# epruesse/metacov

Hardware: AMD Instinct MI355X
Metric: aligned bases/sec into per-position depth vector, 1/2/4/8 MI355X (higher is better)
Workload: dtype int32

## Files before the change

### metacov_amd/csrc/engine.hip

```cpp
#include <hip/hip_ext.h>
#include <hip/hip_runtime.h>

#include <algorithm>
#include <atomic>
#include <cmath>
#include <cstdlib>
#include <cstring>
#include <vector>

#include "../../include/metacov_amd.h"
#include "common.h"
#include "kernels.h"
#include "npstd.h"
#include "capmask.h"

#include <hipcub/hipcub.hpp>

using namespace mc;

#ifndef MC_PLAIN_TILES_PER_CHUNK
#define MC_PLAIN_TILES_PER_CHUNK 4
#endif
constexpr int kPlainTilesPerChunk = MC_PLAIN_TILES_PER_CHUNK;

// ... 105 lines not shown
        hipError_t e = hipHostMalloc(&h, n, hipHostMallocDefault);
        if (e == hipSuccess) cap = n;
        else h = nullptr;
        return e;
    }
    void release() {
        if (h) (void)hipHostFree(h);
        h = nullptr;
        cap = 0;
    }
};

}

struct mc_ctx {
    int device = 0;
    hipStream_t stream = nullptr;
    bool own_stream = false;

    std::vector<int64_t> len, extent, coff;
    DevBuf<int64_t> d_len, d_coff;
    std::vector<int64_t> coff_dev;
    uint64_t coff_dev_gen = ~0ull;

    int64_t n_reads = 0;
    DevBuf<int32_t> d_tid, d_pos, d_span;
    DevBuf<uint32_t> d_gpos;
    bool spans_pending = false;
    DevBuf<int64_t> d_cig_off;
    DevBuf<uint32_t> d_cigar;
    const int64_t* cig_off_ext = nullptr;
    const uint32_t* cigar_ext = nullptr;

    bool prepared = false;
    bool direct = false;
    bool direct_checked = false;
    bool direct_ok = true;
    bool direct_enabled = true;
    int min_span = 0;
    bool direct_retry_full = false;
    unsigned long long direct_gen = 0;
    int direct_halo = 0;
    int direct_halo_used = 0;
    DevBuf<int32_t> d_jidx;
    DevBuf<int32_t> d_fsamp;
    DevBuf<unsigned long long> d_dres;
// ... 53 lines not shown
        int64_t chunk_w = 0, n_chunks = 0;
        std::vector<int64_t> extent, coff;
    } fcache;
    DevBuf<unsigned> d_flow;
    DevBuf<unsigned> d_fhist;
    HostMapped<int> h_fflag;
    DevBuf<unsigned> d_fb_hist;
    DevBuf<RegionAcc> d_fb_acc;
    DevBuf<int32_t> d_fb_list;
    DevBuf<unsigned> d_fb_cnt;
    DevBuf<unsigned> d_kdone;
    int64_t fb_calls = 0;
    bool fb_recent = false;
    int64_t device_recomputes = 0;
    bool fused_clean = false;
    int64_t fused_clean_R = 0;
    bool check_clean = false;
    DevBuf<unsigned long long> d_check;
    int64_t fused_fallbacks = 0;

    hipEvent_t ev[8] = {};
    struct TimingSet {
        hipEvent_t e[4] = {};
        bool prep = false;
        bool pending = false;
    };
    static constexpr int kTimingSets = 4;
    TimingSet ts[kTimingSets];
    int ts_cur = 0;
    HostMapped<unsigned long long> h_done;
    unsigned long long done_seq = 0;
    bool stamp_ok = true;
    int ingest_grid[2] = {0, 0};
    int k2_resident[6] = {};
    size_t k2_resident_lds[6] = {};
    mc_timings t{};
    bool t_cigar = false, t_prep = false, t_depth = false, t_stats = false;
};

static int ctx_use(mc_ctx* ctx) {
    MC_REQUIRE(ctx, MC_E_INVALID, "null ctx");
    HIP_TRY(hipSetDevice(ctx->device));
    return MC_OK;
}

static void invalidate(mc_ctx* ctx) {
    ctx->prepared = false;
    ctx->direct = false;
    ctx->direct_checked = false;
// ... 102 lines not shown
    if (s) {
        ctx->stream = (hipStream_t)s;
        ctx->own_stream = false;
    } else {
        HIP_TRY(hipStreamCreateWithFlags(&ctx->stream, hipStreamNonBlocking));
        ctx->own_stream = true;
    }
    return MC_OK;
}

extern "C" int mc_ctx_device(const mc_ctx* ctx, int* device) {
    MC_REQUIRE(ctx && device, MC_E_INVALID, "null argument");
    *device = ctx->device;
    return MC_OK;
}

extern "C" int mc_set_contigs(mc_ctx* ctx, int32_t n, const int64_t* lengths) {
    if (int rc = ctx_use(ctx)) return rc;
    MC_REQUIRE(n >= 0 && (n == 0 || lengths), MC_E_INVALID, "bad contig table");
    for (int32_t i = 0; i < n; ++i)
        MC_REQUIRE(lengths[i] >= 0 && lengths[i] < (int64_t(1) << 40), MC_E_INVALID,
                   "contig %d: bad length %lld", i, (long long)lengths[i]);
    ctx->len.assign(lengths, lengths + n);
    ctx->direct_ok = true;
    ctx->long_hint = false;
    ctx->n_reads = 0;
    ctx->spans_pending = false;
    ctx->cig_off_ext = nullptr;
    ctx->cigar_ext = nullptr;
    invalidate(ctx);
    HIP_TRY(ctx->d_len.reserve(std::max<int64_t>(n, 1)));
    if (n) HIP_TRY(hipMemcpy(ctx->d_len.p, lengths, n * sizeof(int64_t), hipMemcpyHostToDevice));
    return MC_OK;
}

static int reserve_reads(mc_ctx* ctx, int64_t n_total, bool cigar_mode) {
    const size_t cap = (size_t)round_up(n_total + kPadBatch, kPadBatch);
    if (cap > ctx->d_tid.cap) {
        size_t ncap = std::max(cap, ctx->d_tid.cap * 3 / 2);
        ncap = (size_t)round_up((int64_t)ncap, kPadBatch);
        DevBuf<int32_t> t2, p2, s2;
        HIP_TRY(t2.reserve(ncap));
        HIP_TRY(p2.reserve(ncap));
        HIP_TRY(s2.reserve(ncap));
        if (ctx->n_reads) {
            HIP_TRY(hipMemcpyAsync(t2.p, ctx->d_tid.p, ctx->n_reads * 4, hipMemcpyDeviceToDevice, ctx->stream));
// ... 138 lines not shown
#define MC_STEP_EVENTS 1
#endif
#ifndef MC_EXT_EVENTS
#define MC_EXT_EVENTS 0
#endif
static float elapsed(hipEvent_t a, hipEvent_t b) {
    float ms = 0.f;
    if (hipEventElapsedTime(&ms, a, b) != hipSuccess) {
        (void)hipGetLastError();
        return 0.f;
    }
    return ms;
}

static float elapsed(mc_ctx* ctx, int a, int b) { return elapsed(ctx->ev[a], ctx->ev[b]); }

static void resolve_prepare_timing(mc_ctx* ctx) {
    if (!ctx->prep_pending || hipEventQuery(ctx->ev[3]) != hipSuccess) return;
    ctx->t.prepare_ms = elapsed(ctx, 2, 3);
    ctx->t.prepare_ms_total += ctx->t.prepare_ms;
    ctx->prep_pending = false;
}

static void resolve_timings(mc_ctx* ctx, bool all) {
    for (int i = 1; i <= mc_ctx::kTimingSets; ++i) {
        const int k = (ctx->ts_cur + i) % mc_ctx::kTimingSets;
        auto& T = ctx->ts[k];
        if (!T.pending || (k == ctx->ts_cur && !all)) continue;
        const float a = elapsed(T.e[1], T.e[2]), b = elapsed(T.e[2], T.e[3]);
        ctx->t.fused_depth_ms_total += a;
        ctx->t.fused_stats_ms_total += b;
        ctx->t.depth_ms = a;
        ctx->t.stats_ms = b;
        if (T.prep) {
            ctx->t.prepare_ms = elapsed(T.e[0], T.e[1]);
            ctx->t.prepare_ms_total += ctx->t.prepare_ms;
        }
        T.prep = T.pending = false;
    }
}

#ifndef MC_MIN_CHUNKS
#define MC_MIN_CHUNKS 2048
#endif
static void set_layout(mc_ctx* ctx, const std::vector<int64_t>& ext) {
    const int32_t nc = (int32_t)ctx->len.size();
    ctx->extent = ext;
    ctx->coff.resize(nc + 1);
    int64_t off = 0;
    for (int32_t i = 0; i < nc; ++i) {
        ctx->coff[i] = off;
        off += round_up(ext[i], 64);
    }
    ctx->coff[nc] = off;
    ctx->total_len = off;
    const int64_t tiles = std::max<int64_t>(1, (off + kTileW - 1) / kTileW);
    const int top = ctx->long_hint ? kTilesPerChunkLong : kTilesPerChunk;
    const int min_tpc = (kRing % kTileW == 0) ? kRing / kTileW : top;
    int tpc = top;
    while (tpc / 2 >= min_tpc && tpc % 2 == 0 && tiles / tpc < MC_MIN_CHUNKS &&
           ((int64_t)(tpc / 2) * kTileW) % kRing == 0)
        tpc /= 2;
    ctx->tiles_per_chunk = tpc;
    ctx->chunk_w = (int64_t)tpc * kTileW;
    ctx->n_chunks = std::max<int64_t>(1, (off + ctx->chunk_w - 1) / ctx->chunk_w);
    int tpc_base = tpc;
    if (tpc > kPlainTilesPerChunk && tpc % kPlainTilesPerChunk == 0 &&
        ((int64_t)kPlainTilesPerChunk * kTileW) % kRing == 0)
        tpc_base = kPlainTilesPerChunk;
// ... 209 lines not shown
        HIP_TRY(hipStreamSynchronize(s));
        ctx->t.cigar_ms = elapsed(ctx, 0, 1);
    } else if (ctx->t_cigar) {
        ctx->t.cigar_ms = elapsed(ctx, 0, 1);
    }
    ctx->prep_pending = true;
    ctx->prepared = true;
    ctx->depth_valid = false;
    ++ctx->prep_gen;
    ctx->t.full_prepares += 1;
    return MC_OK;
}

static bool direct_eligible(const mc_ctx* ctx) {
    return ctx->direct_enabled && ctx->direct_ok && ctx->n_reads > 0 && !ctx->len.empty();
}

static int prepare_direct(mc_ctx* ctx) {
    const int32_t nc = (int32_t)ctx->len.size();
    const int64_t n = ctx->n_reads;
    hipStream_t s = ctx->stream;
    if (int rc = run_k1(ctx)) return rc;
    auto& T = ctx->ts[ctx->ts_cur];
    if (MC_STEP_EVENTS && !MC_EXT_EVENTS) HIP_TRY(hipEventRecord(T.e[0], s));
    T.prep = true;
    ctx->ring = kRing;
    ctx->short_max = ctx->ring - kTileW;
    const size_t n_res = 8 + 2 * (size_t)nc;
    HIP_TRY(ctx->pin_io.reserve((n_res + nc + 1) * 8));
    int64_t* coff_up = reinterpret_cast<int64_t*>(static_cast<unsigned long long*>(ctx->pin_io.h) + n_res);
    set_layout(ctx, ctx->len);
    if (int rc = upload_coff(ctx, coff_up)) return rc;
    const int64_t n_base = ctx->n_chunks * ctx->cstride;
    HIP_TRY(ctx->d_jidx.reserve(3 * (n_base + 1)));
    HIP_TRY(ctx->d_fsamp.reserve(nc + 1));
    if (!ctx->d_dres.p) {
        HIP_TRY(ctx->d_dres.reserve(kDresWords));
        HIP_TRY(hipMemsetAsync(ctx->d_dres.p, 0, kDresWords * 8, s));
    }
    ctx->direct_halo_used = ctx->direct_halo > 0 ? std::min(ctx->direct_halo, ctx->short_max) : ctx->short_max;
    ProbeArgs P{ctx->d_tid.p, ctx->d_pos.p, ctx->d_span.p, n, nc, ctx->d_coff.p, base_lw(ctx),
                ctx->short_max, ctx->direct_halo_used, n_base, ctx->d_jidx.p, ctx->d_jidx.p + (n_base + 1),
                ctx->d_jidx.p + 2 * (n_base + 1), ctx->d_fsamp.p,
                ctx->d_dres.p, ++ctx->direct_gen};
    const int64_t M = (n + kProbeStride - 1) >> kProbeShift;
    hipExtLaunchKernelGGL(probe_kernel, dim3((unsigned)std::max<int64_t>(1, (M + kBlock - 1) / kBlock)),
                          dim3(kBlock), 0, s, MC_STEP_EVENTS && MC_EXT_EVENTS ? T.e[0] : nullptr, nullptr, 0, P);
    HIP_TRY(hipGetLastError());
    HIP_TRY(ctx->d_depth.reserve((size_t)(ctx->n_chunks * ctx->chunk_w)));
    ctx->has_long = false;
    ctx->max_span = 0;
    ctx->aligned_bases = -1;
    ctx->prepared = true;
    ctx->direct = true;
    ctx->direct_checked = false;
    ctx->depth_valid = false;
    ++ctx->prep_gen;
    return MC_OK;
}

static int next_halo(unsigned long long max_span, int short_max) {
    const long long h = round_up((long long)max_span + (long long)max_span / 8, 64);
    return (int)std::max<long long>(64, std::min<long long>(h, short_max));
}

static bool check_direct(mc_ctx* ctx, const unsigned long long* res, bool deferred = false) {
    const unsigned long long g = ctx->direct_gen;
    if (res[kDresBadSample] == g || res[kDresLongSample] == g || res[kDresFlags] ||
        res[kDresMaxSpan] > (unsigned long long)ctx->direct_halo_used)
        return false;
    ctx->max_span = (int32_t)res[kDresMaxSpan];
    ctx->direct_halo = next_halo(res[kDresMaxSpan], ctx->short_max);
    ctx->aligned_bases = -1;
    ctx->direct_checked = true;
    ctx->t.direct_batches += 1;
    auto& T = ctx->ts[ctx->ts_cur];
    if (!deferred && T.prep) {
        ctx->t.prepare_ms = elapsed(T.e[0], ctx->ev[4]);
        ctx->t.prepare_ms_total += ctx->t.prepare_ms;
        T.prep = false;
    }
    ctx->t.cigar_ms = ctx->t_cigar ? elapsed(ctx, 0, 1) : 0.f;
    return true;
}

static void direct_fallback(mc_ctx* ctx, const unsigned long long* res) {
    const unsigned long long g = ctx->direct_gen;
    const bool long_reads = res[kDresLongSample] == g || res[kDresMaxSpan] > (unsigned long long)ctx->short_max;
    if (long_reads || (res[kDresFlags] & kDirectUnfit)) ctx->direct_ok = false;
    if (long_reads || res[kDresBadSample] == g || res[kDresFlags]) {
        ctx->direct_retry_full = true;
    } else {
        ctx->direct_halo = next_halo(res[kDresMaxSpan], ctx->short_max);
        ctx->t.halo_redos += 1;
    }
    ctx->fused_clean = false;
    invalidate(ctx);
}

static int prepare_for_compute(mc_ctx* ctx) {
    if (ctx->prepared) return MC_OK;
// ... 62 lines not shown
              "K2Consts: padding beyond DirectArgs' 4 bytes after nc");
static int k2_consts(mc_ctx* ctx, const K2Consts& kc, const K2Consts** out) {
    for (int i = 0; i < mc_ctx::kK2Slots; ++i)
        if (ctx->k2c_valid[i] && std::memcmp(&ctx->k2c[i], &kc, sizeof kc) == 0) {
            *out = ctx->d_k2c.p + i;
            return MC_OK;
        }
    HIP_TRY(ctx->d_k2c.reserve(mc_ctx::kK2Slots));
    HIP_TRY(ctx->h_k2c.reserve(sizeof(K2Consts) * mc_ctx::kK2Slots));
    const int i = ctx->k2c_next;
    ctx->k2c_next = (i + 1) % mc_ctx::kK2Slots;
    if (ctx->k2c_ev[i]) HIP_TRY(hipEventSynchronize(ctx->k2c_ev[i]));
    else HIP_TRY(hipEventCreateWithFlags(&ctx->k2c_ev[i], hipEventDisableTiming));
    K2Consts* stage = reinterpret_cast<K2Consts*>(ctx->h_k2c.h) + i;
    std::memcpy(stage, &kc, sizeof kc);
    HIP_TRY(hipMemcpyAsync(ctx->d_k2c.p + i, stage, sizeof kc, hipMemcpyHostToDevice, ctx->stream));
    HIP_TRY(hipEventRecord(ctx->k2c_ev[i], ctx->stream));
    ctx->k2c[i] = kc;
    ctx->k2c_valid[i] = true;
    *out = ctx->d_k2c.p + i;
    return MC_OK;
}

static int launch_depth(mc_ctx* ctx, const FusedRegions& fr, hipEvent_t ea = nullptr, hipEvent_t eb = nullptr) {
    hipStream_t s = ctx->stream;
    const bool stats = fr.n > 0;
    const size_t lds = (size_t)(kLdsHeader + ctx->ring +
                                (stats ? (ctx->has_long ? HistCfg<true>::kLds : HistCfg<false>::kLds) + kOvInts
                                       : 0)) * 4;
    const bool lng = ctx->has_long;
    const bool dir = ctx->direct;
    const void* kfn = stats ? (lng ? (const void*)depth_kernel<true, true, false>
                                   : dir ? (const void*)depth_kernel<true, false, true>
                                         : (const void*)depth_kernel<true, false, false>)
                            : (lng ? (const void*)depth_kernel<false, true, false>
                                   : dir ? (const void*)depth_kernel<false, false, true>
                                         : (const void*)depth_kernel<false, false, false>);
    const K2Geom geo = k2_geom(ctx, stats);
    const int tpc = geo.tpc;
    const int64_t nch = geo.n_chunks;
    const int cstride = geo.cstride;
    const int64_t* cfirst = ctx->d_chunk_first.p;
    int grid = 0;
    if (int rc = occupancy_grid(ctx, (stats ? 1 : 0) + (lng ? 2 : dir ? 4 : 0), kfn, lds, nch, &grid))
        return rc;
    if (!stats) {
        ctx->fused_clean = false;
        HIP_TRY(hipMemsetAsync(ctx->d_queue.p, 0, 32, s));
        HIP_TRY(hipMemsetAsync(ctx->d_maxdepth.p, 0, 16, s));
    }
    hipEvent_t k2_start = MC_STEP_EVENTS || !ea ? (ea ? ea : ctx->ev[4]) : nullptr;
    hipEvent_t k2_stop = MC_STEP_EVENTS || !eb ? (eb ? eb : ctx->ev[5]) : nullptr;
    if (!MC_EXT_EVENTS && k2_start) HIP_TRY(hipEventRecord(k2_start, s));
    const int64_t* toff = ctx->has_long ? ctx->d_tile_off.p : nullptr;
    const int32_t* tev = ctx->has_long ? ctx->d_tile_ev.p : nullptr;
    const int* ccar = ctx->has_long ? ctx->d_chunk_carry.p : nullptr;
    const int64_t n_base = ctx->n_chunks * ctx->cstride;
    K2Consts kc;
    std::memset(&kc, 0, sizeof kc);
    kc.A = ReadArrays{ctx->d_gpos.p, ctx->d_tid.p, ctx->d_pos.p, ctx->d_span.p};
    kc.R = fr;
    DirectWindow w = direct_window(ctx);
    w.parity = 0;
    kc.D.j0 = ctx->d_jidx.p;
    kc.D.jh = ctx->d_jidx.p + (n_base + 1);
    kc.D.jn = ctx->d_jidx.p + 2 * (n_base + 1);
    kc.D.len = ctx->d_len.p;
    kc.D.nc = (int32_t)ctx->len.size();
    kc.D.dres = ctx->d_dres.p;
    kc.D.win = w;
    const K2Consts* dk = nullptr;
    if (int rc = k2_consts(ctx, kc, &dk)) return rc;
    const int win_parity = (int)(ctx->direct_gen & 1);
#define MC_LAUNCH_K2(S, L, D)                                                                  \
    hipExtLaunchKernelGGL((depth_kernel<S, L, D>), dim3(grid), dim3(kK2Block), (uint32_t)lds, s,        \
// ... 199 lines not shown

struct FusedLayout {
    size_t gs, ge, id, base, ntot, nzx, brow, rtid, rfused, up, total;
};
static FusedLayout fused_layout(int64_t nf, int64_t R) {
    auto al = stage_align;
    FusedLayout L;
    L.gs = 0;
    L.ge = L.gs + al(nf * 8);
    L.id = L.ge + al(nf * 8);
    L.base = L.id + al(nf * 4);
    L.ntot = L.base + al(nf * 4);
    L.nzx = L.ntot + al(R * 8);
    L.brow = L.nzx + al(R * 8);
    L.rtid = L.brow + al(R * 4);
    L.rfused = L.rtid + al(R * 4);
    L.up = L.rfused + al(R * 4);
    L.total = L.up;
    return L;
}

constexpr int kRedo = 1;

static size_t fflag_ints(int64_t R) { return (size_t)round_up(R + 1, 2) + 2 * kDresWords; }
static unsigned long long* fflag_dres(int* base, int64_t R) {
    return reinterpret_cast<unsigned long long*>(base + round_up(R + 1, 2));
}

static int direct_verdict_sync(mc_ctx* ctx) {
    if (!ctx->direct || ctx->direct_checked) return MC_OK;
    unsigned long long* res = static_cast<unsigned long long*>(ctx->pin_io.h);
    HIP_TRY(hipMemcpyAsync(res, ctx->d_dres.p, kDresWords * 8, hipMemcpyDeviceToHost, ctx->stream));
    HIP_TRY(hipStreamSynchronize(ctx->stream));
    if (check_direct(ctx, res)) return MC_OK;
    direct_fallback(ctx, res);
    return kRedo;
}

#ifndef MC_DONE_MODE
#define MC_DONE_MODE 1
#endif
static int wait_event_spin(hipEvent_t ev) {
    for (;;) {
        const hipError_t e = hipEventQuery(ev);
        if (e == hipSuccess) return MC_OK;
        if (e != hipErrorNotReady) HIP_TRY(e);
        __builtin_ia32_pause();
// ... 47 lines not shown
    } else if (ctx->check_clean) {
        HIP_TRY(ctx->d_check.reserve(1));
        HIP_TRY(hipMemsetAsync(ctx->d_check.p, 0, sizeof(unsigned long long), s));
        hipLaunchKernelGGL(fused_clean_check_kernel, dim3(1024), dim3(kBlock), 0, s, ctx->d_fhist.p, R * vals,
                           ctx->d_flow.p, ctx->d_acc.p, R, ctx->d_queue.p, ctx->d_maxdepth.p, ctx->d_check.p);
        HIP_TRY(hipGetLastError());
        unsigned long long bad = 0;
        HIP_TRY(hipMemcpyAsync(&bad, ctx->d_check.p, sizeof bad, hipMemcpyDeviceToHost, s));
        HIP_TRY(hipStreamSynchronize(s));
        MC_REQUIRE(bad == 0, MC_E_STATE, "fused buffers not initialised on a clean call (%llu words differ)", bad);
    }
    FusedRegions fr{nf,
                    ctx->d_fchunk.p,
                    reinterpret_cast<const int64_t*>(d + o_gs),
                    d_fge,
                    reinterpret_cast<const int32_t*>(d + o_id),
                    reinterpret_cast<const int32_t*>(d + o_base),
                    reinterpret_cast<const int32_t*>(d + L.rtid),
                    ctx->d_acc.p,
                    ctx->d_fhist.p,
                    ctx->d_flow.p};
    if (nf == 0) fr.n = 0;
    auto& T = ctx->ts[ctx->ts_cur];
    if (int rc = launch_depth(ctx, fr, T.e[1], T.e[2])) return rc;
    const unsigned long long seq = ++ctx->done_seq;
    unsigned long long* stamp = nullptr;
    if (ctx->stamp_ok) {
        if (!ctx->h_done.h) {
            if (ctx->h_done.reserve(1) != hipSuccess || ctx->d_kdone.reserve(1) != hipSuccess ||
                hipMemsetAsync(ctx->d_kdone.p, 0, sizeof(unsigned), s) != hipSuccess) {
                (void)hipGetLastError();
                ctx->stamp_ok = false;
            } else {
                __atomic_store_n(ctx->h_done.h, 0ull, __ATOMIC_RELEASE);
            }
        }
        if (ctx->stamp_ok && MC_DONE_MODE == 1) stamp = ctx->h_done.d;
    }
    const bool devfb = ctx->has_long || ctx->fb_recent;
    FbArgs F{};
    if (devfb) {
        if (!ctx->d_fb_cnt.p) {
            HIP_TRY(ctx->d_fb_hist.reserve((size_t)kFbSlots * kLdsBins));
            HIP_TRY(ctx->d_fb_acc.reserve(kFbSlots));
            HIP_TRY(ctx->d_fb_list.reserve(kFbSlots));
            HIP_TRY(ctx->d_fb_cnt.reserve(2));
            HIP_TRY(hipMemsetAsync(ctx->d_fb_cnt.p, 0, 8, s));
            hipLaunchKernelGGL(fused_init_kernel, dim3(1024), dim3(kBlock), 0, s, ctx->d_fb_hist.p,
                               (int64_t)kFbSlots * kLdsBins, (unsigned*)nullptr, ctx->d_fb_acc.p,
                               (int64_t)kFbSlots, (const int64_t*)nullptr, (int64_t)0, (int64_t)1, (int64_t)0,
                               (int64_t*)nullptr, (unsigned*)nullptr, (int*)nullptr);
            HIP_TRY(hipGetLastError());
        }
        F = FbArgs{ctx->d_depth.p,
                   reinterpret_cast<const int32_t*>(d + L.rfused),
                   reinterpret_cast<const int64_t*>(d + o_gs),
                   reinterpret_cast<const int64_t*>(d + o_ge),
                   reinterpret_cast<const int64_t*>(d + o_ntot),
                   reinterpret_cast<const int64_t*>(d + o_nzx),
                   ctx->h_fflag.d + R,
                   ctx->d_fb_list.p,
                   ctx->d_fb_cnt.p,
                   (int)(ctx->fb_calls & 1),
                   ctx->d_fb_hist.p,
                   ctx->d_fb_acc.p,
                   d_out};
        ctx->fb_calls += 1;
    }
    hipEvent_t k3_stop = MC_STEP_EVENTS && MC_EXT_EVENTS ? T.e[3] : nullptr;
#define MC_LAUNCH_K3B(V)                                                                           \
    hipExtLaunchKernelGGL(region_final_wave_kernel<V>, dim3((unsigned)((R + kWaves - 1) / kWaves)),     \
                          dim3(kBlock), 0u, s, nullptr, devfb ? nullptr : k3_stop, 0u,                   \
                          ctx->d_fhist.p, R, ctx->d_acc.p,                                              \
                       reinterpret_cast<const int64_t*>(d + o_ntot),                                \
                       reinterpret_cast<const int64_t*>(d + o_nzx), d_out, ctx->h_fflag.d,           \
                       reinterpret_cast<const int32_t*>(d + o_brow), ctx->d_flow.p,                 \
                       ctx->d_maxdepth.p, ctx->h_fflag.d + R, ctx->d_queue.p,                       \
                       verdict ? ctx->d_dres.p : nullptr, verdict ? fflag_dres(ctx->h_fflag.d, R) : nullptr, \
                       devfb ? F.cnt + F.parity : nullptr, devfb ? F.list : nullptr,                \
                       ctx->direct ? direct_window(ctx) : DirectWindow{},                          \
                       ctx->direct ? reinterpret_cast<const int32_t*>(d + L.rtid) : nullptr,           \
                       ctx->d_kdone.p, devfb ? nullptr : stamp, seq)
    if (vals == HistCfg<false>::kBins) MC_LAUNCH_K3B(HistCfg<false>::kBins);
    else MC_LAUNCH_K3B(HistCfg<true>::kBins);
#undef MC_LAUNCH_K3B
    HIP_TRY(hipGetLastError());
    if (devfb) {
        hipLaunchKernelGGL(fb_seg_kernel, dim3(1024), dim3(kBlock), (size_t)kLdsBins * 4, s, F);
        HIP_TRY(hipGetLastError());
        hipExtLaunchKernelGGL(fb_final_kernel, dim3(kFbSlots), dim3(kBlock), 0u, s, nullptr, k3_stop, 0u, F);
        HIP_TRY(hipGetLastError());
    }
    if (MC_STEP_EVENTS && !MC_EXT_EVENTS) HIP_TRY(hipEventRecord(T.e[3], s));
    if ((MC_DONE_MODE == 0 || (MC_DONE_MODE == 1 && devfb)) && ctx->stamp_ok && hipStreamWriteValue64(s, ctx->h_done.d, seq, 0) != hipSuccess) {
        (void)hipGetLastError();
        ctx->stamp_ok = false;
    }
    ctx->t_stats = false;
    ctx->t.stats_launches += 1;
    resolve_timings(ctx, false);
    if (int rc = MC_DONE_MODE == 2 ? wait_event_spin(T.e[3]) : wait_stamp(ctx, seq)) return rc;
    const int* flags = ctx->h_fflag.h;
    if (verdict && !check_direct(ctx, fflag_dres(ctx->h_fflag.h, R), true)) {
        direct_fallback(ctx, fflag_dres(ctx->h_fflag.h, R));
        T.prep = T.pending = false;
        return kRedo;
    }
    T.pending = true;
    ctx->ts_cur = (ctx->ts_cur + 1) % mc_ctx::kTimingSets;
    ctx->max_depth = flags[R];
    int64_t n_flag = 0;
    for (int64_t r = 0; r < R; ++r) n_flag += flags[r] ? 1 : 0;
    const bool on_device = devfb && n_flag <= kFbSlots && ctx->max_depth < kLdsBins;
    std::vector<int32_t> ft;
    std::vector<int64_t> fs, fe, fr_idx;
    if (!on_device)
        for (int64_t r = 0; r < R; ++r)
            if (flags[r]) {
                ft.push_back(tid[r]);
                fs.push_back(start[r]);
                fe.push_back(end[r]);
                fr_idx.push_back(r);
            }
    ctx->fused_fallbacks = (int64_t)ft.size();
    ctx->device_recomputes = on_device ? n_flag : 0;
    ctx->fb_recent = n_flag > 0;
    if (ft.empty()) {
        ctx->fused_clean = true;
        ctx->fused_clean_R = R;
    }
    if (!ft.empty()) {
        if (int rc = region_stats_impl(ctx, (int64_t)ft.size(), ft.data(), fs.data(), fe.data(),
                                       d_out, fr_idx.data()))
            return rc;
        HIP_TRY(hipEventSynchronize(ctx->ev[7]));
        ctx->t.fused_stats_ms_total += elapsed(ctx, 6, 7);
    }
    ctx->t.fused_calls += 1;
    return MC_OK;
}

static int depth_stats_once(mc_ctx* ctx, int64_t R, const int32_t* tid, const int64_t* start,
                            const int64_t* end, RegionOut* d_out) {
    if (int rc = prepare_for_compute(ctx)) return rc;
    MC_REQUIRE(R >= 0 && (R == 0 || (tid && start && end)), MC_E_INVALID, "bad region arrays");
    auto& fc = ctx->fcache;
    const bool direct = ctx->direct;
    const int vals = fused_hist_vals(ctx->has_long);
    const int64_t win_below = (int64_t)kWinBelow * vals / kHistBins;
    const double span_mean = ctx->n_reads ? (double)ctx->aligned_bases / (double)ctx->n_reads : 0.0;
    auto window_base = [&](int32_t t) {
        const int64_t ext = ctx->extent[t];
        const double body = ext > 2 * span_mean ? (double)ext - span_mean : (double)ext;
        const double depth_est = ext > 0 ? (double)ctx->cbases[t] / body : 0.0;
        return (int32_t)std::max<int64_t>(0, std::llrint(depth_est) - win_below);
    };
    const bool same = R > 0 && fc.valid && (int64_t)fc.tid.size() == R &&
                      std::memcmp(fc.tid.data(), tid, R * 4) == 0 &&
                      std::memcmp(fc.start.data(), start, R * 8) == 0 &&
                      std::memcmp(fc.end.data(), end, R * 8) == 0;
    if (same && fc.gen == ctx->prep_gen) return depth_stats_launch(ctx, R, tid, start, end, d_out, fc.nf);
    const K2Geom geo = k2_geom(ctx, true);
    if (same && fc.vals == vals && fc.chunk_w == geo.chunk_w && fc.n_chunks == geo.n_chunks &&
        fc.extent == ctx->extent && fc.coff == ctx->coff) {
        const FusedLayout L = fused_layout(fc.nf, R);
        if (!direct && R > 0) {
            const int32_t nc = (int32_t)ctx->len.size();
// ... 403 lines not shown
```

### metacov_amd/csrc/kernels.h

```cpp
#pragma once

#include <hip/hip_runtime.h>
#include <stdint.h>

namespace mc {

#ifndef MC_TILE_W
#define MC_TILE_W 4096
#endif
#ifndef MC_RING
#define MC_RING (2 * MC_TILE_W)
#endif
#ifndef MC_TILES_PER_CHUNK
#define MC_TILES_PER_CHUNK 8
#endif
#ifndef MC_PREFETCH
#define MC_PREFETCH 1
#endif
#ifndef MC_PREFETCH_STATS
#define MC_PREFETCH_STATS 1
#endif
#ifndef MC_APPLY_SHORT
#define MC_APPLY_SHORT 1
#endif
// ... 504 lines not shown
    if (threadIdx.x < 4) {
        long long v = red[threadIdx.x][0];
#pragma unroll
        for (int w = 1; w < kWaves; ++w)
            v = threadIdx.x == 3 ? max(v, red[3][w]) : v + red[threadIdx.x][w];
        if (threadIdx.x == 3) atomicMax(&out[3], (unsigned long long)v);
        else if (v) atomicAdd(&out[threadIdx.x], (unsigned long long)v);
    }
}

constexpr int kProbeShift = 8;
constexpr int kNearHalo = 256;
constexpr int kFarHaloMin = MC_FAR_HALO_MIN;
constexpr int kProbeStride = 1 << kProbeShift;

enum : int {
    kDresBadSample = 0,
    kDresLongSample = 1,
    kDresFlags = 2,
    kDresBases = 3,
    kDresMaxSpan = 4,
    kDresSpanSum = 5,
    kDresSpanCnt = 6,
    kDresWords = 9
};
constexpr unsigned kDirectInvalid = 1;
constexpr unsigned kDirectUnfit = 2;

struct ProbeArgs {
    const int32_t* tid;
    const int32_t* pos;
    const int32_t* span;
    int64_t n;
    int32_t nc;
    const int64_t* coff;
    int lw;
    int short_max;
    int halo;
    int64_t n_base;
    int32_t* j0;
    int32_t* jh;
    int32_t* jn;
    int32_t* fsamp;
    unsigned long long* dres;
    unsigned long long gen;
};

struct DirectWindow {
// ... 21 lines not shown

__device__ __forceinline__ int64_t probe_key(const ProbeArgs& A, int t, int p) {
    const int ct = t < 0 ? 0 : t >= A.nc ? A.nc - 1 : t;
    const int64_t k = A.coff[ct] + (int64_t)(p < 0 ? 0 : p);
    return k;
}

__device__ __forceinline__ void probe_fill(int32_t* J, int64_t n_base, int lw, int64_t off, int64_t key,
                                           int64_t key_next, bool first, bool last, int32_t val) {
    int64_t k0 = first ? 0 : ((key + off) >> lw) + 1;
    int64_t k1 = last ? n_base : ((key_next + off) >> lw);
    if (k1 > n_base) k1 = n_base;
    if (first) {
        int64_t kz = (key + off) >> lw;
        if (kz > n_base) kz = n_base;
        for (int64_t k = 0; k <= kz; ++k) J[k] = 0;
        k0 = kz + 1;
    }
    for (int64_t k = k0; k <= k1; ++k) J[k] = val;
}

constexpr int kProbeSpanEvery = 4;
constexpr unsigned kProbeMeanBlocks = 64;

__global__ void __launch_bounds__(kBlock)
probe_kernel(ProbeArgs A) {
    const int64_t M = (A.n + kProbeStride - 1) >> kProbeShift;
    const int64_t j = (int64_t)blockIdx.x * kBlock + threadIdx.x;
    const int par = (int)(A.gen & 1);
    if (blockIdx.x == 0 && threadIdx.x >= kDresFlags && threadIdx.x <= kDresMaxSpan) A.dres[threadIdx.x] = 0;
    if (blockIdx.x == 0 && threadIdx.x < 2) A.dres[kDresSpanSum + 2 * (par ^ 1) + threadIdx.x] = 0;
    const bool sampled = j < M && (j % kProbeSpanEvery) == 0;
    const int s0 = sampled ? A.span[j << kProbeShift] : 0;
    const unsigned every = max(1u, gridDim.x / kProbeMeanBlocks);
    if (blockIdx.x % every == 0) {
        __shared__ long long red[2 * kWaves];
        const bool s_ok = sampled && s0 >= 0;
        const long long wsum = wave_sum64(s_ok ? (long long)s0 : 0);
        const long long wcnt = wave_sum64(s_ok ? 1 : 0);
        if ((threadIdx.x & 63) == 0) {
            red[threadIdx.x >> 6] = wsum;
            red[kWaves + (threadIdx.x >> 6)] = wcnt;
        }
        __syncthreads();
        if (threadIdx.x == 0) {
            long long ts = 0, tc = 0;
#pragma unroll
            for (int w = 0; w < kWaves; ++w) {
                ts += red[w];
                tc += red[kWaves + w];
            }
            if (tc) {
                atomicAdd(&A.dres[kDresSpanSum + 2 * par], (unsigned long long)ts);
                atomicAdd(&A.dres[kDresSpanCnt + 2 * par], (unsigned long long)tc);
            }
        }
    }
    if (j >= M) return;
    const bool last = j == M - 1;
    const int64_t i = j << kProbeShift, i1 = last ? i : i + kProbeStride;
    const int t = A.tid[i], p = A.pos[i];
    const int t_next = A.tid[i1], p_next = A.pos[i1];
    const int s = s0;
    const int64_t key = probe_key(A, t, p);
    const int64_t key_next = probe_key(A, t_next, p_next);
    const bool bad = ((unsigned)t >= (unsigned)A.nc) | (p < 0) | (s < 0);
    const bool uns = !last && ((t > t_next) | ((t == t_next) & (p > p_next)) | (key > key_next));
    if (bad | uns) atomicMax(&A.dres[kDresBadSample], A.gen);
    if (s > A.short_max) atomicMax(&A.dres[kDresLongSample], A.gen);
    const bool first = j == 0;
    probe_fill(A.j0, A.n_base, A.lw, 0, key, key_next, first, last, (int32_t)(j + 1));
    probe_fill(A.jh, A.n_base, A.lw, A.halo, key, key_next, first, last, (int32_t)(j + 1));
    if (MC_FAR_HALO) probe_fill(A.jn, A.n_base, A.lw, kNearHalo, key, key_next, first, last, (int32_t)(j + 1));
    const int ct = t < 0 ? 0 : t >= A.nc ? A.nc - 1 : t;
    const int cn = last ? A.nc : (t_next < 0 ? 0 : t_next >= A.nc ? A.nc - 1 : t_next);
    if (first)
        for (int k = 0; k <= ct; ++k) A.fsamp[k] = 0;
    for (int k = ct + 1; k <= cn; ++k) A.fsamp[k] = (int32_t)(j + 1);
}

__global__ void __launch_bounds__(kBlock)
window_bases_kernel(const unsigned long long* __restrict__ ingest_out, const unsigned long long* __restrict__ cbases,
                    int64_t n, const int64_t* __restrict__ len, const int32_t* __restrict__ rtid,
                    const int32_t* __restrict__ rfused, int64_t R, int win_below, int32_t* __restrict__ brow,
                    int32_t* __restrict__ fbase) {
// ... 753 lines not shown
    unsigned f = a.flags;
    int m = a.max_span;
#pragma unroll
    for (int d = 32; d > 0; d >>= 1) {
        f |= __shfl_xor(f, d, 64);
        m = max(m, __shfl_xor(m, d, 64));
    }
    __syncthreads();
    if (lane == 0) {
        red[wave] = (int)f;
        red[kK2Waves + wave] = m;
    }
    __syncthreads();
    if (threadIdx.x == 0) {
        unsigned ff = 0;
        int mm = 0;
#pragma unroll
        for (int w = 0; w < kK2Waves; ++w) {
            ff |= (unsigned)red[w];
            mm = max(mm, red[kK2Waves + w]);
        }
        if (ff) atomicOr(&D.dres[kDresFlags], (unsigned long long)ff);
        if (mm > 0) atomicMax(&D.dres[kDresMaxSpan], (unsigned long long)mm);
    }
}

__global__ void __launch_bounds__(kBlock)
span_sum_kernel(const int32_t* __restrict__ span, int64_t n, unsigned long long* __restrict__ part) {
    long long s = 0;
    const int64_t n4 = n >> 2;
    const int64_t stride = (int64_t)gridDim.x * kBlock;
    int64_t i = (int64_t)blockIdx.x * kBlock + threadIdx.x;
    for (; i + 3 * stride < n4; i += 4 * stride) {
        i32x4 v[4];
#pragma unroll
        for (int u = 0; u < 4; ++u) v[u] = __builtin_nontemporal_load(reinterpret_cast<const i32x4*>(span) + i + u * stride);
#pragma unroll
        for (int u = 0; u < 4; ++u) s += (long long)v[u].x + v[u].y + v[u].z + v[u].w;
    }
    for (; i < n4; i += stride) {
        const i32x4 v = reinterpret_cast<const i32x4*>(span)[i];
        s += (long long)v.x + v.y + v.z + v.w;
    }
    if (blockIdx.x == 0 && threadIdx.x < (n & 3)) s += span[(n4 << 2) + threadIdx.x];
    s = wave_sum64(s);
    __shared__ long long ws[kWaves];
// ... 235 lines not shown
             int32_t* __restrict__ depth, unsigned* __restrict__ queue,
             int* __restrict__ max_depth, unsigned long long gen, int win_parity) {
    static_assert(!(kDirect && kLong), "the direct path has no long reads");
    const auto& KC = *(const __attribute__((address_space(4))) K2Consts*)K;
    const auto& R = KC.R;
    const auto& D = KC.D;
    extern __shared__ __attribute__((aligned(16))) int lds[];
    int* hdr = lds;
    int and_flip = 0;
    int* ring = lds + kLdsHeader;
    unsigned* hist = reinterpret_cast<unsigned*>(ring + kRing);
    using HC = HistCfg<kLong>;
    OvLds* ovf = reinterpret_cast<OvLds*>(hist + HC::kLds);
    const int lane = threadIdx.x & 63;
    unsigned* hist_lane = hist + (lane & (HC::kCopies - 1)) * HC::kStride;
    const int hist_dummy = HC::kBins + (lane / HC::kCopies) % HC::kPad;
    const int wave = __builtin_amdgcn_readfirstlane(threadIdx.x >> 6);
    const int64_t chunk_w = (int64_t)tiles_per_chunk * kTileW;
    constexpr int kWaveSpan = kTileW / kK2Waves;
    constexpr int kChunks = kWaveSpan / (64 * 4);
    constexpr bool kDefer = !kStats || (kLong && MC_DEFER_LONG) || (kDirect && MC_DEFER_DIRECT);
    constexpr bool kPf = kStats ? MC_PREFETCH_STATS : MC_PREFETCH;
    if (kDirect) {
        const unsigned long long f0 = uload(D.dres, kDresBadSample), f1 = uload(D.dres, kDresLongSample);
        if (f0 == gen || f1 == gen) return;
    }
    int my_max = 0;
    DirectAcc dacc;
    OvReg ovr;
    ov_reg_reset(ovr);
    if (kStats) {
        for (int k = threadIdx.x; k < HC::kLds; k += kK2Block) hist[k] = 0;
        if (threadIdx.x < kOvRecs) ov_reset(ovf + threadIdx.x);
    }

    constexpr bool kAhead = kStats && kLong;
    int ticket = 0;
    if (threadIdx.x == 0) hdr[0] = take_chunk(queue, n_chunks);
    const int ring_tail = (int)(((int64_t)tiles_per_chunk * kTileW) % kRing);
    for (int k = threadIdx.x * 4; k < kRing; k += kK2Block * 4)
        *reinterpret_cast<i32x4*>(ring + k) = i32x4{0, 0, 0, 0};
    for (;;) {
        __syncthreads();
        const int64_t c = (unsigned)__builtin_amdgcn_readfirstlane(hdr[0]);
        if (c >= n_chunks) break;
        if (kAhead && threadIdx.x == 0) ticket = take_chunk(queue, n_chunks);
// ... 555 lines not shown
            vmax = max(vmax, max(max(y0, y1), max(y2, y3)));
            vmin = min(vmin, min(min((unsigned)y0, (unsigned)y1), min((unsigned)y2, (unsigned)y3)));
        }
    }
}

struct FbArgs {
    const int32_t* depth;
    const int32_t* rfused;
    const int64_t* fgs;
    const int64_t* fge;
    const int64_t* ntot;
    const int64_t* nzx;
    const int* max_depth;
    int32_t* list;
    unsigned* cnt;
    int parity;
    unsigned* hist;
    RegionAcc* acc;
    RegionOut* out;
};

__device__ __forceinline__ void grid_done_stamp(unsigned* done_cnt, unsigned long long* stamp,
                                                unsigned long long seq) {
    if (stamp == nullptr) return;
    asm volatile("s_waitcnt vmcnt(0)" ::: "memory");
    __syncthreads();
    if (threadIdx.x == 0) {
        const unsigned prev = __hip_atomic_fetch_add(done_cnt, 1u, __ATOMIC_RELAXED, __HIP_MEMORY_SCOPE_AGENT);
        if (prev == gridDim.x - 1) {
            __hip_atomic_store(done_cnt, 0u, __ATOMIC_RELAXED, __HIP_MEMORY_SCOPE_AGENT);
            __builtin_amdgcn_fence(__ATOMIC_RELEASE, "");
            __hip_atomic_store(stamp, seq, __ATOMIC_RELAXED, __HIP_MEMORY_SCOPE_SYSTEM);
        }
    }
}

template <class T>
__device__ __forceinline__ void store_sys(T* p, T v) {
    __hip_atomic_store(p, v, __ATOMIC_RELAXED, __HIP_MEMORY_SCOPE_SYSTEM);
}

__global__ void __launch_bounds__(kBlock)
fb_seg_kernel(FbArgs F) {
    extern __shared__ __attribute__((aligned(16))) unsigned hb[];
    const int n = (int)min(F.cnt[F.parity], (unsigned)kFbSlots);
    const int maxd = *F.max_depth;
    if (n == 0 || maxd >= kLdsBins) return;
    const int nb = maxd + 1;
    const int per = max(1, (int)gridDim.x / n);
    __shared__ int ext[2 * kWaves];
    for (int w = blockIdx.x; w < n * per; w += gridDim.x) {
        const int i = w / per, part = w % per;
        const int k = F.rfused[F.list[i]];
// ... 46 lines not shown
        F.acc[b].min = 0x7fffffff;
        F.acc[b].max = 0;
    }
}

__global__ void __launch_bounds__(kBlock)
fb_final_kernel(FbArgs F) {
    fb_final_row(F);
}

template <int kVals>
__device__ __forceinline__ void
final_wave_row(unsigned* __restrict__ hist, int64_t R,
               RegionAcc* __restrict__ acc, const int64_t* __restrict__ n_total,
               const int64_t* __restrict__ n_zero_extra, RegionOut* __restrict__ out,
               int* __restrict__ fallback, const int32_t* __restrict__ base_of,
               unsigned* __restrict__ low_of, int* __restrict__ max_depth,
               int* __restrict__ max_out, unsigned* __restrict__ queue,
               const unsigned long long* __restrict__ dres_in, unsigned long long* __restrict__ dres_out,
               unsigned* __restrict__ fb_cnt, int32_t* __restrict__ fb_list,
               DirectWindow dwin, const int32_t* __restrict__ rtid, bool wt) {
    constexpr int kFinPer = (kVals + 63) / 64;
    const int lane = threadIdx.x & 63;
    if (blockIdx.x == 0 && dres_out && threadIdx.x < kDresWords) {
        if (wt) store_sys(dres_out + threadIdx.x, dres_in[threadIdx.x]);
        else dres_out[threadIdx.x] = dres_in[threadIdx.x];
    }
    if (blockIdx.x == 0 && threadIdx.x == 0) {
        if (max_out) {
            if (wt) store_sys(max_out, *max_depth);
            else *max_out = *max_depth;
        }
        if (queue) {
            for (int k = 0; k < 4; ++k) max_depth[k] = 0;
            for (int k = 0; k < 8; ++k) queue[k] = 0;
        }
    }
    const int64_t r = (int64_t)blockIdx.x * kWaves + (threadIdx.x >> 6);
    if (r >= R) return;
    unsigned* hr = hist + r * kVals;
    const long long n = n_total[r];
    const long long zx = n_zero_extra[r];
    const long long base = rtid ? direct_window_base(dwin, dwin.parity, __builtin_amdgcn_readfirstlane(rtid[r]))
                                : base_of[r];
    const long long zx_bin = base == 0 ? zx : 0;
    const long long low = (long long)low_of[r] + (base == 0 ? 0 : zx);
    const long long r_lo = (n - 1) / 2, r_hi = n / 2;
// ... 98 lines not shown
        const unsigned long long* v = reinterpret_cast<const unsigned long long*>(&o);
#pragma unroll
        for (int k = 0; k < (int)(sizeof(RegionOut) / 8); ++k) store_sys(w + k, v[k]);
    } else {
        out[r] = o;
    }
}

template <int kVals>
__global__ void __launch_bounds__(kBlock)
region_final_wave_kernel(unsigned* __restrict__ hist, int64_t R,
                         RegionAcc* __restrict__ acc, const int64_t* __restrict__ n_total,
                         const int64_t* __restrict__ n_zero_extra, RegionOut* __restrict__ out,
                         int* __restrict__ fallback, const int32_t* __restrict__ base_of,
                         unsigned* __restrict__ low_of, int* __restrict__ max_depth,
                         int* __restrict__ max_out, unsigned* __restrict__ queue,
                         const unsigned long long* __restrict__ dres_in, unsigned long long* __restrict__ dres_out,
                         unsigned* __restrict__ fb_cnt, int32_t* __restrict__ fb_list,
                         DirectWindow dwin, const int32_t* __restrict__ rtid,
                         unsigned* __restrict__ done_cnt, unsigned long long* __restrict__ stamp,
                         unsigned long long seq) {
    final_wave_row<kVals>(hist, R, acc, n_total, n_zero_extra, out, fallback, base_of, low_of, max_depth,
                          max_out, queue, dres_in, dres_out, fb_cnt, fb_list, dwin, rtid, stamp != nullptr);
    grid_done_stamp(done_cnt, stamp, seq);
}

}
```

Before: 14450 billion.

## Replace per-call timing events with device wall clocks and skip redundant layout upload

```diff
diff --git a/metacov_amd/csrc/engine.hip b/metacov_amd/csrc/engine.hip
--- a/metacov_amd/csrc/engine.hip
+++ b/metacov_amd/csrc/engine.hip
@@ -151,6 +151,10 @@
     DevBuf<int64_t> d_len, d_coff;
     std::vector<int64_t> coff_dev;
     uint64_t coff_dev_gen = ~0ull;
+    uint64_t layout_gen = 0;
+    uint64_t direct_layout_gen = ~0ull;
+    uint64_t direct_coff_gen = ~0ull;
+    bool direct_layout_long = false;
 
     int64_t n_reads = 0;
     DevBuf<int32_t> d_tid, d_pos, d_span;
@@ -250,9 +254,13 @@
     hipEvent_t ev[8] = {};
     struct TimingSet {
         hipEvent_t e[4] = {};
+        unsigned long long clk[4] = {};
         bool prep = false;
         bool pending = false;
+        bool by_clock = false;
     };
+    bool clock_call = false;
+    double clk_khz = 0;
     static constexpr int kTimingSets = 4;
     TimingSet ts[kTimingSets];
     int ts_cur = 0;
@@ -401,6 +409,7 @@
         MC_REQUIRE(lengths[i] >= 0 && lengths[i] < (int64_t(1) << 40), MC_E_INVALID,
                    "contig %d: bad length %lld", i, (long long)lengths[i]);
     ctx->len.assign(lengths, lengths + n);
+    ++ctx->layout_gen;
     ctx->direct_ok = true;
     ctx->long_hint = false;
     ctx->n_reads = 0;
@@ -585,21 +594,26 @@
     ctx->prep_pending = false;
 }
 
+static float clock_ms(const mc_ctx* ctx, unsigned long long a, unsigned long long b) {
+    return b > a && ctx->clk_khz > 0 ? (float)((double)(b - a) / ctx->clk_khz) : 0.f;
+}
+
 static void resolve_timings(mc_ctx* ctx, bool all) {
     for (int i = 1; i <= mc_ctx::kTimingSets; ++i) {
         const int k = (ctx->ts_cur + i) % mc_ctx::kTimingSets;
         auto& T = ctx->ts[k];
         if (!T.pending || (k == ctx->ts_cur && !all)) continue;
-        const float a = elapsed(T.e[1], T.e[2]), b = elapsed(T.e[2], T.e[3]);
+        const float a = T.by_clock ? clock_ms(ctx, T.clk[1], T.clk[2]) : elapsed(T.e[1], T.e[2]);
+        const float b = T.by_clock ? clock_ms(ctx, T.clk[2], T.clk[3]) : elapsed(T.e[2], T.e[3]);
         ctx->t.fused_depth_ms_total += a;
         ctx->t.fused_stats_ms_total += b;
         ctx->t.depth_ms = a;
         ctx->t.stats_ms = b;
         if (T.prep) {
-            ctx->t.prepare_ms = elapsed(T.e[0], T.e[1]);
+            ctx->t.prepare_ms = T.by_clock ? clock_ms(ctx, T.clk[0], T.clk[1]) : elapsed(T.e[0], T.e[1]);
             ctx->t.prepare_ms_total += ctx->t.prepare_ms;
         }
-        T.prep = T.pending = false;
+        T.prep = T.pending = T.by_clock = false;
     }
 }
 
@@ -608,6 +622,7 @@
 #endif
 static void set_layout(mc_ctx* ctx, const std::vector<int64_t>& ext) {
     const int32_t nc = (int32_t)ctx->len.size();
+    ++ctx->layout_gen;
     ctx->extent = ext;
     ctx->coff.resize(nc + 1);
     int64_t off = 0;
@@ -863,21 +878,28 @@
     hipStream_t s = ctx->stream;
     if (int rc = run_k1(ctx)) return rc;
     auto& T = ctx->ts[ctx->ts_cur];
-    if (MC_STEP_EVENTS && !MC_EXT_EVENTS) HIP_TRY(hipEventRecord(T.e[0], s));
+    T.by_clock = ctx->clock_call;
+    if (MC_STEP_EVENTS && !MC_EXT_EVENTS && !T.by_clock) HIP_TRY(hipEventRecord(T.e[0], s));
     T.prep = true;
     ctx->ring = kRing;
     ctx->short_max = ctx->ring - kTileW;
     const size_t n_res = 8 + 2 * (size_t)nc;
     HIP_TRY(ctx->pin_io.reserve((n_res + nc + 1) * 8));
-    int64_t* coff_up = reinterpret_cast<int64_t*>(static_cast<unsigned long long*>(ctx->pin_io.h) + n_res);
-    set_layout(ctx, ctx->len);
-    if (int rc = upload_coff(ctx, coff_up)) return rc;
+    if (ctx->direct_layout_gen != ctx->layout_gen || ctx->direct_layout_long != ctx->long_hint ||
+        ctx->direct_coff_gen != ctx->d_coff.gen || ctx->coff_dev_gen != ctx->d_coff.gen) {
+        int64_t* coff_up = reinterpret_cast<int64_t*>(static_cast<unsigned long long*>(ctx->pin_io.h) + n_res);
+        set_layout(ctx, ctx->len);
+        if (int rc = upload_coff(ctx, coff_up)) return rc;
+        ctx->direct_layout_gen = ctx->layout_gen;
+        ctx->direct_layout_long = ctx->long_hint;
+        ctx->direct_coff_gen = ctx->d_coff.gen;
+    }
     const int64_t n_base = ctx->n_chunks * ctx->cstride;
     HIP_TRY(ctx->d_jidx.reserve(3 * (n_base + 1)));
     HIP_TRY(ctx->d_fsamp.reserve(nc + 1));
     if (!ctx->d_dres.p) {
-        HIP_TRY(ctx->d_dres.reserve(kDresWords));
-        HIP_TRY(hipMemsetAsync(ctx->d_dres.p, 0, kDresWords * 8, s));
+        HIP_TRY(ctx->d_dres.reserve(kDresTotal));
+        HIP_TRY(hipMemsetAsync(ctx->d_dres.p, 0, kDresTotal * 8, s));
     }
     ctx->direct_halo_used = ctx->direct_halo > 0 ? std::min(ctx->direct_halo, ctx->short_max) : ctx->short_max;
     ProbeArgs P{ctx->d_tid.p, ctx->d_pos.p, ctx->d_span.p, n, nc, ctx->d_coff.p, base_lw(ctx),
@@ -917,7 +939,7 @@
     ctx->t.direct_batches += 1;
     auto& T = ctx->ts[ctx->ts_cur];
     if (!deferred && T.prep) {
-        ctx->t.prepare_ms = elapsed(T.e[0], ctx->ev[4]);
+        ctx->t.prepare_ms = T.by_clock ? 0.f : elapsed(T.e[0], ctx->ev[4]);
         ctx->t.prepare_ms_total += ctx->t.prepare_ms;
         T.prep = false;
     }
@@ -1026,7 +1048,8 @@
     return MC_OK;
 }
 
-static int launch_depth(mc_ctx* ctx, const FusedRegions& fr, hipEvent_t ea = nullptr, hipEvent_t eb = nullptr) {
+static int launch_depth(mc_ctx* ctx, const FusedRegions& fr, hipEvent_t ea = nullptr, hipEvent_t eb = nullptr,
+                        bool no_events = false) {
     hipStream_t s = ctx->stream;
     const bool stats = fr.n > 0;
     const size_t lds = (size_t)(kLdsHeader + ctx->ring +
@@ -1053,8 +1076,8 @@
         HIP_TRY(hipMemsetAsync(ctx->d_queue.p, 0, 32, s));
         HIP_TRY(hipMemsetAsync(ctx->d_maxdepth.p, 0, 16, s));
     }
-    hipEvent_t k2_start = MC_STEP_EVENTS || !ea ? (ea ? ea : ctx->ev[4]) : nullptr;
-    hipEvent_t k2_stop = MC_STEP_EVENTS || !eb ? (eb ? eb : ctx->ev[5]) : nullptr;
+    hipEvent_t k2_start = !no_events && (MC_STEP_EVENTS || !ea) ? (ea ? ea : ctx->ev[4]) : nullptr;
+    hipEvent_t k2_stop = !no_events && (MC_STEP_EVENTS || !eb) ? (eb ? eb : ctx->ev[5]) : nullptr;
     if (!MC_EXT_EVENTS && k2_start) HIP_TRY(hipEventRecord(k2_start, s));
     const int64_t* toff = ctx->has_long ? ctx->d_tile_off.p : nullptr;
     const int32_t* tev = ctx->has_long ? ctx->d_tile_ev.p : nullptr;
@@ -1300,7 +1323,7 @@
 
 constexpr int kRedo = 1;
 
-static size_t fflag_ints(int64_t R) { return (size_t)round_up(R + 1, 2) + 2 * kDresWords; }
+static size_t fflag_ints(int64_t R) { return (size_t)round_up(R + 1, 2) + 2 * kDresTotal; }
 static unsigned long long* fflag_dres(int* base, int64_t R) {
     return reinterpret_cast<unsigned long long*>(base + round_up(R + 1, 2));
 }
@@ -1394,7 +1417,6 @@
                     ctx->d_flow.p};
     if (nf == 0) fr.n = 0;
     auto& T = ctx->ts[ctx->ts_cur];
-    if (int rc = launch_depth(ctx, fr, T.e[1], T.e[2])) return rc;
     const unsigned long long seq = ++ctx->done_seq;
     unsigned long long* stamp = nullptr;
     if (ctx->stamp_ok) {
@@ -1410,6 +1432,10 @@
         if (ctx->stamp_ok && MC_DONE_MODE == 1) stamp = ctx->h_done.d;
     }
     const bool devfb = ctx->has_long || ctx->fb_recent;
+    const bool clk = MC_CLOCK_TIMINGS && verdict && stamp && !devfb && ctx->clk_khz > 0 && (!T.prep || T.by_clock);
+    if (T.prep && T.by_clock && !clk) T.prep = false;
+    T.by_clock = clk;
+    if (int rc = launch_depth(ctx, fr, T.e[1], T.e[2], clk)) return rc;
     FbArgs F{};
     if (devfb) {
         if (!ctx->d_fb_cnt.p) {
@@ -1439,7 +1465,7 @@
                    d_out};
         ctx->fb_calls += 1;
     }
-    hipEvent_t k3_stop = MC_STEP_EVENTS && MC_EXT_EVENTS ? T.e[3] : nullptr;
+    hipEvent_t k3_stop = MC_STEP_EVENTS && MC_EXT_EVENTS && !clk ? T.e[3] : nullptr;
 #define MC_LAUNCH_K3B(V)                                                                           \
     hipExtLaunchKernelGGL(region_final_wave_kernel<V>, dim3((unsigned)((R + kWaves - 1) / kWaves)),     \
                           dim3(kBlock), 0u, s, nullptr, devfb ? nullptr : k3_stop, 0u,                   \
@@ -1463,7 +1489,7 @@
         hipExtLaunchKernelGGL(fb_final_kernel, dim3(kFbSlots), dim3(kBlock), 0u, s, nullptr, k3_stop, 0u, F);
         HIP_TRY(hipGetLastError());
     }
-    if (MC_STEP_EVENTS && !MC_EXT_EVENTS) HIP_TRY(hipEventRecord(T.e[3], s));
+    if (MC_STEP_EVENTS && !MC_EXT_EVENTS && !clk) HIP_TRY(hipEventRecord(T.e[3], s));
     if ((MC_DONE_MODE == 0 || (MC_DONE_MODE == 1 && devfb)) && ctx->stamp_ok && hipStreamWriteValue64(s, ctx->h_done.d, seq, 0) != hipSuccess) {
         (void)hipGetLastError();
         ctx->stamp_ok = false;
@@ -1475,8 +1501,12 @@
     const int* flags = ctx->h_fflag.h;
     if (verdict && !check_direct(ctx, fflag_dres(ctx->h_fflag.h, R), true)) {
         direct_fallback(ctx, fflag_dres(ctx->h_fflag.h, R));
-        T.prep = T.pending = false;
+        T.prep = T.pending = T.by_clock = false;
         return kRedo;
+    }
+    if (clk) {
+        const unsigned long long* w = fflag_dres(ctx->h_fflag.h, R);
+        for (int k = 0; k < 4; ++k) T.clk[k] = __atomic_load_n(w + kDresClkProbe + k, __ATOMIC_RELAXED);
     }
     T.pending = true;
     ctx->ts_cur = (ctx->ts_cur + 1) % mc_ctx::kTimingSets;
@@ -1514,7 +1544,18 @@
 
 static int depth_stats_once(mc_ctx* ctx, int64_t R, const int32_t* tid, const int64_t* start,
                             const int64_t* end, RegionOut* d_out) {
-    if (int rc = prepare_for_compute(ctx)) return rc;
+    if (MC_CLOCK_TIMINGS && ctx->clk_khz == 0) {
+        int khz = 0;
+        if (hipDeviceGetAttribute(&khz, hipDeviceAttributeWallClockRate, ctx->device) != hipSuccess) {
+            (void)hipGetLastError();
+            khz = 0;
+        }
+        ctx->clk_khz = khz > 0 ? (double)khz : -1.0;
+    }
+    ctx->clock_call = MC_CLOCK_TIMINGS && MC_DONE_MODE == 1 && ctx->stamp_ok && ctx->clk_khz > 0 && !ctx->fb_recent;
+    const int prc = prepare_for_compute(ctx);
+    ctx->clock_call = false;
+    if (prc) return prc;
     MC_REQUIRE(R >= 0 && (R == 0 || (tid && start && end)), MC_E_INVALID, "bad region arrays");
     auto& fc = ctx->fcache;
     const bool direct = ctx->direct;
diff --git a/metacov_amd/csrc/kernels.h b/metacov_amd/csrc/kernels.h
--- a/metacov_amd/csrc/kernels.h
+++ b/metacov_amd/csrc/kernels.h
@@ -550,8 +550,16 @@
     kDresMaxSpan = 4,
     kDresSpanSum = 5,
     kDresSpanCnt = 6,
-    kDresWords = 9
+    kDresWords = 9,
+    kDresClkProbe = 9,
+    kDresClkK2Start = 10,
+    kDresClkK2End = 11,
+    kDresClkK3End = 12,
+    kDresTotal = 13
 };
+#ifndef MC_CLOCK_TIMINGS
+#define MC_CLOCK_TIMINGS 1
+#endif
 constexpr unsigned kDirectInvalid = 1;
 constexpr unsigned kDirectUnfit = 2;
 
@@ -619,12 +627,18 @@
 
 constexpr int kProbeSpanEvery = 4;
 constexpr unsigned kProbeMeanBlocks = 64;
+#ifndef MC_PROBE_SPARSE
+#define MC_PROBE_SPARSE 1
+#endif
+constexpr int kProbeTidEvery = 4;
+static_assert(64 % kProbeTidEvery == 0 && kBlock % 64 == 0, "anchors are lanes: a group must not straddle a wave");
 
 __global__ void __launch_bounds__(kBlock)
 probe_kernel(ProbeArgs A) {
     const int64_t M = (A.n + kProbeStride - 1) >> kProbeShift;
     const int64_t j = (int64_t)blockIdx.x * kBlock + threadIdx.x;
     const int par = (int)(A.gen & 1);
+    if (MC_CLOCK_TIMINGS && blockIdx.x == 0 && threadIdx.x == 0) A.dres[kDresClkProbe] = wall_clock64();
     if (blockIdx.x == 0 && threadIdx.x >= kDresFlags && threadIdx.x <= kDresMaxSpan) A.dres[threadIdx.x] = 0;
     if (blockIdx.x == 0 && threadIdx.x < 2) A.dres[kDresSpanSum + 2 * (par ^ 1) + threadIdx.x] = 0;
     const bool sampled = j < M && (j % kProbeSpanEvery) == 0;
@@ -653,11 +667,40 @@
             }
         }
     }
+    if (M <= 0) return;
+    const bool last = j == M - 1;
+    int t, p, t_next, p_next;
+    if (MC_PROBE_SPARSE) {
+        const int64_t jc = j < M ? j : M - 1, jx = jc + 1 < M ? jc + 1 : M - 1;
+        const int64_t i = jc << kProbeShift, i1 = jx << kProbeShift;
+        const int lane = threadIdx.x & 63;
+        const bool anchor = (lane & (kProbeTidEvery - 1)) == 0;
+        p = A.pos[i];
+        const int ta = anchor ? A.tid[i] : 0;
+        int tn = 0, pn = 0;
+        if (lane == 63) {
+            tn = A.tid[i1];
+            pn = A.pos[i1];
+        }
+        const int g0 = lane & ~(kProbeTidEvery - 1);
+        const int t_lo = __shfl(ta, g0, 64);
+        const int t_in = __shfl(ta, (g0 + kProbeTidEvery) & 63, 64), t_63 = __shfl(tn, 63, 64);
+        const int t_hi = g0 + kProbeTidEvery == 64 ? t_63 : t_in;
+        t = t_lo;
+        if (!anchor && t_lo != t_hi) t = A.tid[i];
+        t_next = __shfl_down(t, 1, 64);
+        p_next = __shfl_down(p, 1, 64);
+        if (lane == 63) {
+            t_next = tn;
+            p_next = pn;
+        }
+    } else {
+        const int64_t jc = j < M ? j : M - 1;
+        const int64_t i = jc << kProbeShift, i1 = jc >= M - 1 ? i : i + kProbeStride;
+        t = A.tid[i], p = A.pos[i];
+        t_next = A.tid[i1], p_next = A.pos[i1];
+    }
     if (j >= M) return;
-    const bool last = j == M - 1;
-    const int64_t i = j << kProbeShift, i1 = last ? i : i + kProbeStride;
-    const int t = A.tid[i], p = A.pos[i];
-    const int t_next = A.tid[i1], p_next = A.pos[i1];
     const int s = s0;
     const int64_t key = probe_key(A, t, p);
     const int64_t key_next = probe_key(A, t_next, p_next);
@@ -1457,6 +1500,7 @@
         }
         if (ff) atomicOr(&D.dres[kDresFlags], (unsigned long long)ff);
         if (mm > 0) atomicMax(&D.dres[kDresMaxSpan], (unsigned long long)mm);
+        if (MC_CLOCK_TIMINGS) atomicMax(&D.dres[kDresClkK2End], (unsigned long long)wall_clock64());
     }
 }
 
@@ -1738,6 +1782,7 @@
     constexpr bool kDefer = !kStats || (kLong && MC_DEFER_LONG) || (kDirect && MC_DEFER_DIRECT);
     constexpr bool kPf = kStats ? MC_PREFETCH_STATS : MC_PREFETCH;
     if (kDirect) {
+        if (MC_CLOCK_TIMINGS && blockIdx.x == 0 && threadIdx.x == 0) D.dres[kDresClkK2Start] = wall_clock64();
         const unsigned long long f0 = uload(D.dres, kDresBadSample), f1 = uload(D.dres, kDresLongSample);
         if (f0 == gen || f1 == gen) return;
     }
@@ -2339,7 +2384,7 @@
 };
 
 __device__ __forceinline__ void grid_done_stamp(unsigned* done_cnt, unsigned long long* stamp,
-                                                unsigned long long seq) {
+                                                unsigned long long seq, unsigned long long* clk_end = nullptr) {
     if (stamp == nullptr) return;
     asm volatile("s_waitcnt vmcnt(0)" ::: "memory");
     __syncthreads();
@@ -2347,6 +2392,9 @@
         const unsigned prev = __hip_atomic_fetch_add(done_cnt, 1u, __ATOMIC_RELAXED, __HIP_MEMORY_SCOPE_AGENT);
         if (prev == gridDim.x - 1) {
             __hip_atomic_store(done_cnt, 0u, __ATOMIC_RELAXED, __HIP_MEMORY_SCOPE_AGENT);
+            if (clk_end)
+                __hip_atomic_store(clk_end, (unsigned long long)wall_clock64(), __ATOMIC_RELAXED,
+                                   __HIP_MEMORY_SCOPE_SYSTEM);
             __builtin_amdgcn_fence(__ATOMIC_RELEASE, "");
             __hip_atomic_store(stamp, seq, __ATOMIC_RELAXED, __HIP_MEMORY_SCOPE_SYSTEM);
         }
@@ -2439,7 +2487,7 @@
                DirectWindow dwin, const int32_t* __restrict__ rtid, bool wt) {
     constexpr int kFinPer = (kVals + 63) / 64;
     const int lane = threadIdx.x & 63;
-    if (blockIdx.x == 0 && dres_out && threadIdx.x < kDresWords) {
+    if (blockIdx.x == 0 && dres_out && threadIdx.x < (MC_CLOCK_TIMINGS ? kDresClkK3End : kDresWords)) {
         if (wt) store_sys(dres_out + threadIdx.x, dres_in[threadIdx.x]);
         else dres_out[threadIdx.x] = dres_in[threadIdx.x];
     }
@@ -2584,7 +2632,7 @@
                          unsigned long long seq) {
     final_wave_row<kVals>(hist, R, acc, n_total, n_zero_extra, out, fallback, base_of, low_of, max_depth,
                           max_out, queue, dres_in, dres_out, fb_cnt, fb_list, dwin, rtid, stamp != nullptr);
-    grid_done_stamp(done_cnt, stamp, seq);
-}
-
-}
+    grid_done_stamp(done_cnt, stamp, seq, MC_CLOCK_TIMINGS && dres_out ? dres_out + kDresClkK3End : nullptr);
+}
+
+}
```

New measurement: 14660 billion, median of 6. 1.4% higher.
